# yzang2019/tendermint-fork

Hardware: AMD Instinct MI355X
Metric: ed25519 verifies/sec at 1/8 MI355X (higher is better)
Workload: dtype u32 (GF(2^255-19) radix 2^25.5 limbs, int64 accumulate); 1 GPU; C2: raw batch of 1048576 ed25519 signatures per GPU; signatures_per_gpu=1048576, key_cache=False, parallelism=shard-per-gpu x1

## Files before the change

### include/tmed25519.h

```cpp
#ifndef TMED25519_H
#define TMED25519_H

#include <stddef.h>
#include <stdint.h>

#ifdef __cplusplus
extern "C" {
#endif

#define TMED_OK 0
#define TMED_EINVAL (-1)
#define TMED_ENODEV (-2)
#define TMED_EHIP (-3)
#define TMED_ENOMEM (-4)
#define TMED_ENOKEYSET (-5)
#define TMED_EINTERNAL (-6)

typedef struct tmed_ctx tmed_ctx;

int tmed_device_count(void);

int tmed_init(int device, tmed_ctx **out);
void tmed_destroy(tmed_ctx *ctx);
const char *tmed_strerror(int code);
// ... 35 lines not shown
                                    const uint8_t *d_msgs, const uint32_t *d_msg_off, size_t n, uint8_t *d_out_valid,
                                    void *stream);


int tmed_verify_batch_zip215(tmed_ctx *ctx, const uint8_t *pubkeys, const uint8_t *sigs, const uint32_t *sig_lens,
                             const uint8_t *msgs, const uint32_t *msg_off, size_t n, uint8_t *out_valid);
int tmed_verify_batch_zip215_device(tmed_ctx *ctx, const uint8_t *d_pubkeys, const uint8_t *d_sigs,
                                    const uint8_t *d_msgs, const uint32_t *d_msg_off, size_t n, uint8_t *d_out_valid,
                                    void *stream);
int tmed_zip215_set_seed(const uint8_t *seed32);
int tmed_zip215_stats(uint32_t out[4]);


typedef struct {
  const char *chain_id;
  uint32_t chain_id_len;
  int64_t height;
  int32_t round;
  const uint8_t *block_hash;
  uint32_t block_hash_len;
  uint32_t psh_total;
  const uint8_t *psh_hash;
  uint32_t psh_hash_len;
} tmed_vote_template;

int tmed_vote_sign_bytes(const tmed_vote_template *t, size_t n, const uint8_t *flags, const int64_t *ts_seconds,
                         const int32_t *ts_nanos, uint8_t *out, size_t out_cap, uint32_t *out_off, size_t *out_len);


int tmed_valu_peak(tmed_ctx *ctx, int kind, double *giga_ops_per_s);

void tmed_test_pool_jitter(int max_us);
void tmed_test_stream_delay(int us);

int tmed_debug_zero_bits(void *out, size_t cap, size_t *n);


typedef struct {
  const uint8_t *hash;
  uint32_t hash_len;
  uint32_t psh_total;
  const uint8_t *psh_hash;
  uint32_t psh_hash_len;
} tmed_block_id;

typedef struct {
  size_t n;
  const uint8_t *pubkeys;
  const int64_t *powers;
  const uint8_t *addresses;
  int64_t total_power;
  uint64_t keyset;
  const uint32_t *keyset_index;
  const uint8_t *set_hash;
} tmed_valset;

typedef struct {
  int64_t height;
  int32_t round;
  tmed_block_id block_id;
  size_t n_sigs;
  const uint8_t *flags;
  const uint8_t *addresses;
  const int64_t *ts_seconds;
  const int32_t *ts_nanos;
  const uint8_t *sigs;
// ... 223 lines not shown
```

### tendermint-fork_amd/csrc/kernels.h

```cpp
#pragma once
#include <hip/hip_runtime.h>
#include <stddef.h>
#include <stdint.h>

#include "ge25519.h"
#include "signbytes.h"

namespace tmed {

struct KernelTimer {
  static constexpr int kMax = 160;
  hipEvent_t ev[kMax];
  int kind[kMax];
  int n = 0;
  void mark(hipStream_t s, int k) {
    if (n < kMax) { kind[n] = k; (void)hipEventRecord(ev[n++], s); }
  }
};

constexpr uint32_t kThreadsPerBlock = 256;
constexpr uint32_t kSlabSlotBytes = 8 * 128;
inline uint32_t slab_tables(int main_waves) { return main_waves == 5 ? 1u : 2u; }

constexpr uint32_t kFinCap = 1u << 20;
constexpr int kFinInt4 = 8;
constexpr uint32_t kFinGroupMax = 16;
constexpr uint32_t kFinPreStride = kFinCap + 64;
constexpr size_t kFinBytes = (size_t)kFinCap * kFinInt4 * 16;
constexpr size_t kFinPreBytes = (size_t)kFinPreStride * 3 * 16;

struct BTabs {
  const int4 *b16;
  const int4 *comb16;
  const int4 *b26 = nullptr;
};
constexpr uint32_t kB26Entries = (1u << 25) + 1;
constexpr size_t kB26Bytes = 2 * (size_t)kB26Entries * 128;
hipError_t launch_build_b26(const int4 *comb16, int4 *tab, hipStream_t stream);
constexpr int kB24Windows = 11;
constexpr uint32_t kB24Entries = (1u << 23) + 1;
constexpr size_t kB24Bytes = (size_t)kB24Windows * kB24Entries * 128;
hipError_t launch_build_b24(const int4 *comb16, int4 *tab, hipStream_t stream);
constexpr uint32_t kB16Entries = 32769;
constexpr size_t kB16Bytes = (size_t)kB16Entries * 128;
hipError_t launch_build_b16(int4 *tab, hipStream_t stream);
constexpr size_t kBComb16Bytes = 16 * kB16Bytes;
void host_bcomb16_bases(int32_t out[16 * 40]);
hipError_t launch_build_bcomb16(const int32_t *d_bases, int4 *comb, hipStream_t stream);

hipError_t launch_verify(const uint8_t *pub, const uint8_t *sig, const uint8_t *msgs, const uint32_t *off,
                         uint32_t n, uint8_t *out, int4 *slab, uint32_t slab_stride, BTabs btab,
                         int4 *prep, int4 *fin, int4 *fin_pre, hipStream_t stream, uint32_t chunk = 0,
                         int main_waves = 6, bool msg_slots = false, KernelTimer *timer = nullptr,
                         bool zip215 = false);

// ... 17 lines not shown
constexpr uint32_t kKeyChunksMax = (1u << 24) >> kKeyChunkBits;

hipError_t launch_comb_bases(const uint8_t *pubs, uint32_t n, int negate, uint8_t *ok, int32_t *bases,
                             hipStream_t stream);
hipError_t launch_comb_fill(const int32_t *bases, uint32_t n, int4 *comb, hipStream_t stream);
#ifndef TMED_COMBA_BITS
#define TMED_COMBA_BITS 12
#endif
constexpr int kCombABits = TMED_COMBA_BITS;
constexpr int kCombAWindows = 253 / kCombABits;
constexpr int kCombATopField = 253 - kCombABits * (kCombAWindows - 1);
constexpr uint32_t kCombAEntries = (1u << (kCombABits - 1)) + 1;
constexpr uint32_t kCombATopMax = (1u << (kCombATopField - 1)) + 1;
constexpr uint32_t kCombATopGroups = (kCombATopMax + 127) / 128;
constexpr uint32_t kCombATopEntries = kCombATopGroups * 128 + 1;
static_assert(kCombABits >= 10 && kCombABits <= 12 && kCombATopField >= kCombABits, "comb radix");
constexpr size_t kCombARowsPerKey = (size_t)(kCombAWindows - 1) * kCombAEntries + kCombATopEntries;
constexpr size_t kCombABytesPerKey = kCombARowsPerKey * kCombEntryInt4 * 16;
constexpr size_t comba_row(int w, uint32_t j) { return (size_t)w * kCombAEntries + j; }
hipError_t launch_build_comba(const uint8_t *pubs, uint32_t n, int32_t *bases, int4 *comba, hipStream_t stream);
hipError_t launch_verify_keyset(const uint32_t *val_idx, uint32_t nkeys, const uint8_t *key_pub, const uint8_t *key_ok,
                                const int4 *const *acomb, const int4 *bcomb, const uint8_t *sig, const uint8_t *msgs,
                                const uint32_t *off, uint32_t n, uint8_t *out, int4 *prep, uint32_t stride,
                                int4 *fin, int4 *fin_pre, hipStream_t stream, bool msg_slots = false,
                                KernelTimer *timer = nullptr, uint32_t *perm = nullptr,
                                uint32_t *order_scratch = nullptr, const int4 *bcomb24 = nullptr,
                                const int4 *const *acomba = nullptr);
constexpr uint32_t kKeyOrderMaxKeys = 1u << 24;
uint32_t key_order_scratch_words(uint32_t n, uint32_t nkeys);
hipError_t launch_key_order(const uint32_t *val_idx, uint32_t n, uint32_t nkeys, uint32_t *scratch, uint32_t *perm,
                            uint32_t index_base, hipStream_t stream);

hipError_t launch_test_delay(hipStream_t stream, uint32_t us);
hipError_t launch_window_stats(const int4 *prep, uint32_t stride, uint32_t count, uint32_t *d_hist,
                               hipStream_t stream);

constexpr uint32_t kLatMax = 1u << 16;
struct VoteAsm;
hipError_t launch_verify_keyset_lat(const uint32_t *val_idx, uint32_t nkeys, const uint8_t *key_pub, const uint8_t *key_ok,
                                    const int4 *const *acomb, const int4 *bcomb, const uint8_t *sig, const uint8_t *msgs,
                                    const uint32_t *off, uint32_t n, uint8_t *out, int4 *fin, int4 *dec,
                                    hipStream_t stream, bool msg_slots = false, const VoteAsm *va = nullptr);

constexpr uint32_t kGLatMax = 1u << 16;
constexpr size_t kGLatHandBytes = (size_t)kGLatMax * (6 * 2 + 7) * 16;
struct VoteAsm {
  const uint8_t *tmpl;
  const uint32_t *tmpl_idx;
  const uint8_t *flags;
  const int64_t *ts_sec;
  const int32_t *ts_nanos;
};

hipError_t launch_verify_glat(const uint8_t *pub, const uint8_t *sig, const uint8_t *msgs, const uint32_t *off,
                              uint32_t n, uint8_t *out, const int4 *comb16, int4 *hand, hipStream_t stream,
                              bool msg_slots = false, KernelTimer *timer = nullptr, const VoteAsm *va = nullptr);

hipError_t launch_assemble_votes(const uint8_t *tmpl, const uint32_t *tmpl_idx, const uint8_t *flags,
                                 const int64_t *ts_sec, const int32_t *ts_nanos, uint32_t n, uint8_t *out,
                                 uint32_t *out_len, hipStream_t stream);

}
```

### tendermint-fork_amd/csrc/kernels.hip

```cpp
#include "kernels.h"
#include "verify_core.h"
#include "verify_hs.h"
#include "kernel_util.h"
#include "rows.h"
#include "votes_dev.h"

namespace tmed {

__device__ int4 kIdentityRow[8] = {{1, 0, 0, 0}, {0, 0, 0, 0}, {1, 0, 0, 0}, {0, 0, 0, 0},
                                          {1, 0, 0, 0}, {0, 0, 0, 0}, {0, 0, 0, 0}, {0, 0, 0, 0}};

__device__ __forceinline__ void slab_st(int4 *p, int4 v) { *p = v; }
__device__ __forceinline__ int4 slab_ld(const int4 *p) { return *p; }

struct SlabTab {
  int4 *base;
  uint32_t slot;

  __device__ __forceinline__ const int4 *row(int j) const {
    return j == 0 ? kIdentityRow : base + ((size_t)slot * 8 + (j - 1)) * 8;
  }

  __device__ __forceinline__ void store(int j, const ge_cached &c) const {
    if (j == 0) return;
    int4 *r = base + ((size_t)slot * 8 + (j - 1)) * 8;
    const fe *fs[4] = {&c.YpX, &c.YmX, &c.Z, &c.T2d};
#pragma unroll
    for (int f = 0; f < 4; f++) {
      uint32_t w[8];
      fe_pack256(w, *fs[f]);
      slab_st(r + 2 * f, make_int4((int)w[0], (int)w[1], (int)w[2], (int)w[3]));
      slab_st(r + 2 * f + 1, make_int4((int)w[4], (int)w[5], (int)w[6], (int)w[7]));
    }
  }
  int4 pv[8];
  __device__ __forceinline__ void prefetch(int j, bool swap = false) {
    const int4 *r = row(j);
    const int sx = swap ? 2 : 0;
#pragma unroll
    for (int q = 0; q < 8; q++) pv[q] = slab_ld(r + (q < 4 ? (q ^ sx) : q));
  }
  __device__ __forceinline__ void take(ge_cached &c) const {
    fe *fs[4] = {&c.YpX, &c.YmX, &c.Z, &c.T2d};
#pragma unroll
    for (int f = 0; f < 4; f++) {
      const uint32_t w[8] = {(uint32_t)pv[2 * f].x, (uint32_t)pv[2 * f].y, (uint32_t)pv[2 * f].z,
                             (uint32_t)pv[2 * f].w, (uint32_t)pv[2 * f + 1].x, (uint32_t)pv[2 * f + 1].y,
                             (uint32_t)pv[2 * f + 1].z, (uint32_t)pv[2 * f + 1].w};
      fe_unpack256(*fs[f], w);
    }
  }
};

typedef __attribute__((address_space(1))) void global_void;
typedef __attribute__((address_space(3))) void lds_void;

template <int BITS>
struct BPf {
  static constexpr int kBits = BITS;
  const int4 *tab;
  int4 *buf;
  uint32_t lane;
  __device__ __forceinline__ void prefetch(int j) const {
    __builtin_amdgcn_s_waitcnt(0xc07f);
#pragma unroll
    for (int q = 0; q < 8; q++)
      __builtin_amdgcn_global_load_lds((global_void *)(tab + (size_t)j * 8 + q), (lds_void *)(buf + q * 64), 16, 0, 0);
  }
  __device__ __forceinline__ void take(ge_niels &e) const { niels_load(e, buf + lane, 64); }
};

constexpr uint32_t kHsBlock = kThreadsPerBlock;

constexpr int kPrepWaves = 3;
__global__ __launch_bounds__(kHsBlock, kPrepWaves) void verify_prep_kernel(
    const uint8_t *__restrict__ pub, const uint8_t *__restrict__ sig, MsgSrc ms, uint32_t base, uint32_t count,
    int4 *__restrict__ prep, uint32_t stride, uint32_t *__restrict__ place) {
  const uint32_t slot = blockIdx.x * blockDim.x + threadIdx.x;
  if (place && slot == 0) place[0] = place[1] = 0;
  if (slot >= count) return;
  const uint32_t i = base + slot;
  uint32_t pw[8];
  bool sok;
  {
    uint32_t sw[16], k[8], h[16];
// ... 163 lines not shown
    const int4 v = active ? prep2[(size_t)q * stride + slot] : make_int4(0, 0, 0, 0);
    w[4 * q] = v.x; w[4 * q + 1] = v.y; w[4 * q + 2] = v.z; w[4 * q + 3] = v.w;
  }
  uint32_t er[8];
#pragma unroll
  for (int j = 0; j < 8; j++) er[j] = (uint32_t)w[13 + j];
  if (BB == 16) {
    uint32_t e[8];
#pragma unroll
    for (int j = 0; j < 8; j++) e[j] = er[j];
    sc_recode_b<16>(er, e);
  }
  fe Rx, Ry;
#pragma unroll
  for (int j = 0; j < 10; j++) { Rx.v[j] = w[21 + j]; Ry.v[j] = w[31 + j]; }
  ge_p3 A;
#pragma unroll
  for (int j = 0; j < 10; j++) { A.X.v[j] = w[44 + j]; A.Y.v[j] = w[54 + j]; }
  if (!active) { fe_1(A.Y); fe_1(Ry); }
  fe_1(A.Z);
  fe_mul(A.T, A.X, A.Y);
  const int flags = w[41];
  int W = active ? (flags >> 8) : 29;
#pragma unroll
  for (int o = 32; o > 0; o >>= 1) {
    const int x = __shfl_xor(W, o);
    W = x > W ? x : W;
  }
  W = __builtin_amdgcn_readfirstlane(W);
  if (W < 29) W = 29;
  if (W > 64) W = 64;
  const uint32_t lane = threadIdx.x & 63u, wv = threadIdx.x >> 6;
  const HsDigitsDev ds{prep2, stride, slot, active};
  SlabTab ta{slab, slot};
  SlabTab tr{slab + (size_t)stride * 64, slot};
  const size_t hi = BB == 26 ? (size_t)kB26Entries * kCombEntryInt4 : (size_t)8 * kB16Entries * kCombEntryInt4;
  BPf<BB> bl{btab, sbl[wv], lane};
  BPf<BB> bh{btab + hi, sbh[wv], lane};
  const bool id = verify_main_hs(ds, (flags & 2) != 0, er, W, A, Rx, Ry, ta, tr, bl, bh, zip215 != 0);
  if (active) out[base + (uint32_t)w[42]] = ((flags & 1) && id) ? 1 : 0;
}

__global__ __launch_bounds__(kThreadsPerBlock) void window_stats_kernel(const int4 *__restrict__ prep2, uint32_t stride,
                                                                       uint32_t count, uint32_t *__restrict__ lane_hist,
                                                                       uint32_t *__restrict__ wave_hist) {
  __shared__ uint32_t lh[65], wh[65];
  for (uint32_t b = threadIdx.x; b < 65; b += blockDim.x) lh[b] = wh[b] = 0;
  __syncthreads();
  const uint32_t slot = blockIdx.x * blockDim.x + threadIdx.x;
  const bool active = slot < count;
  int W = active ? (prep2[(size_t)10 * stride + slot].y >> 8) : 0;
  if (W < 0 || W > 64) W = 64;
  if (active) atomicAdd(&lh[W], 1u);
  int m = W;
#pragma unroll
  for (int o = 32; o > 0; o >>= 1) {
    const int x = __shfl_xor(m, o);
    m = x > m ? x : m;
  }
  if ((threadIdx.x & 63u) == 0 && slot < count) atomicAdd(&wh[m], 1u);
  __syncthreads();
  for (uint32_t b = threadIdx.x; b < 65; b += blockDim.x) {
    if (lh[b]) atomicAdd(&lane_hist[b], lh[b]);
    if (wh[b]) atomicAdd(&wave_hist[b], wh[b]);
  }
}

__global__ __launch_bounds__(64) void test_delay_kernel(uint32_t iters) {
  for (uint32_t i = 0; i < iters; i++) __builtin_amdgcn_s_sleep(127);
}

hipError_t launch_test_delay(hipStream_t stream, uint32_t us) {
  if (us == 0) return hipSuccess;
  hipLaunchKernelGGL(test_delay_kernel, dim3(1), dim3(64), 0, stream, (us < 100000u ? us : 100000u) / 3u + 1u);
  return hipGetLastError();
}

hipError_t launch_window_stats(const int4 *prep, uint32_t stride, uint32_t count, uint32_t *d_hist,
                               hipStream_t stream) {
  if (count == 0) return hipSuccess;
  hipError_t e = hipMemsetAsync(d_hist, 0, 2 * 65 * sizeof(uint32_t), stream);
  if (e != hipSuccess) return e;
  hipLaunchKernelGGL(window_stats_kernel, dim3((count + kThreadsPerBlock - 1) / kThreadsPerBlock),
                     dim3(kThreadsPerBlock), 0, stream, prep + (size_t)kPrepInt4 * stride, stride, count, d_hist,
                     d_hist + 65);
  return hipGetLastError();
}

struct FinDev {
  const int4 *fin;
  int4 *pre;
  const uint8_t *sig;
  uint8_t *out;
  uint32_t fin_base, lane, L, m;
  const uint32_t *perm;
  __device__ __forceinline__ int count() const { return lane < m ? (int)((m - lane + L - 1) / L) : 0; }
  __device__ __forceinline__ uint32_t slot(int j) const { return lane + (uint32_t)j * L; }
  __device__ __forceinline__ void load_z(int j, fe &z) const {
// ... 697 lines not shown
```

### tendermint-fork_amd/csrc/tmed_capi.hip

```cpp
#include <hip/hip_runtime.h>
#include <stdlib.h>
#include <string.h>

#include <algorithm>
#include <map>
#include <mutex>
#include <new>
#include <string>

#include "../../include/tmed25519.h"
#include "kernels.h"

#include "ctx.h"
#include "median_host.h"

using namespace tmed;

extern "C" {

int tmed_device_count(void) {
  int n = 0;
  if (hipGetDeviceCount(&n) != hipSuccess) return 0;
  return n;
}
// ... 88 lines not shown

int tmed_init(int device, tmed_ctx **out) {
  if (!out) return TMED_EINVAL;
  *out = nullptr;
  int ndev = tmed_device_count();
  if (device < 0 || device >= ndev) return TMED_ENODEV;
  hipDeviceProp_t prop;
  if (hipGetDeviceProperties(&prop, device) != hipSuccess) return TMED_EHIP;
  if (strncmp(prop.gcnArchName, "gfx950", 6) != 0) return TMED_ENODEV;
  if (hipSetDevice(device) != hipSuccess) return TMED_EHIP;
  tmed_ctx *c = new tmed_ctx();
  c->device = device;
  hipError_t e = hipStreamCreateWithFlags(&c->stream, hipStreamNonBlocking);
  if (e == hipSuccess) e = hipStreamCreateWithFlags(&c->copy_stream, hipStreamNonBlocking);
  if (e == hipSuccess) e = hipEventCreate(&c->ev0);
  if (e == hipSuccess) e = hipEventCreate(&c->ev1);
  if (e == hipSuccess) e = hipEventCreateWithFlags(&c->scratch_ev, hipEventDisableTiming);
  auto round_up = [](uint32_t v) {
    if (v < kThreadsPerBlock) v = kThreadsPerBlock;
    if (v > (1u << 24)) v = 1u << 24;
    return (v + kThreadsPerBlock - 1) / kThreadsPerBlock * kThreadsPerBlock;
  };
  c->slab_slots = 4096 * kThreadsPerBlock;
  c->chunk = c->slab_slots;
  if (const char *v = getenv("TMED_SLAB_SLOTS")) c->slab_slots = round_up((uint32_t)strtoul(v, nullptr, 10));
  c->chunk = c->slab_slots;
  if (const char *v = getenv("TMED_CHUNK")) c->chunk = std::min(c->slab_slots, round_up((uint32_t)strtoul(v, nullptr, 10)));
  if (const char *v = getenv("TMED_MAIN_WAVES")) c->main_waves = atoi(v) == 5 ? 5 : 6;
  if (const char *v = getenv("TMED_LAT_MAX")) c->lat_max = (uint32_t)strtoul(v, nullptr, 10);
  if (c->lat_max > kLatMax) c->lat_max = kLatMax;
  if (const char *v = getenv("TMED_GLAT_MAX")) c->glat_max = (uint32_t)strtoul(v, nullptr, 10);
  if (c->glat_max > kGLatMax) c->glat_max = kGLatMax;
  if (e == hipSuccess)
    e = hipMalloc((void **)&c->d_slab, (size_t)c->slab_slots * kSlabSlotBytes * slab_tables(c->main_waves));
  if (e == hipSuccess) e = hipMalloc((void **)&c->d_prep, (size_t)c->slab_slots * kPrepSlotBytes + kPrepTailBytes);
  if (e == hipSuccess) e = hipMalloc((void **)&c->d_fin, kFinBytes);
  if (e == hipSuccess) e = hipMalloc((void **)&c->d_fin_pre, kFinPreBytes);
  if (e == hipSuccess) e = hipMalloc((void **)&c->d_glat, kGLatHandBytes);
  uint8_t *d_bpub = nullptr, *d_bok = nullptr;
  const uint8_t benc[32] = {0x58, 0x66, 0x66, 0x66, 0x66, 0x66, 0x66, 0x66, 0x66, 0x66, 0x66,
                            0x66, 0x66, 0x66, 0x66, 0x66, 0x66, 0x66, 0x66, 0x66, 0x66, 0x66,
                            0x66, 0x66, 0x66, 0x66, 0x66, 0x66, 0x66, 0x66, 0x66, 0x66};
  if (e == hipSuccess) e = hipMalloc((void **)&c->d_b16, kB16Bytes);
  if (e == hipSuccess) e = launch_build_b16(c->d_b16, c->stream);
  if (e == hipSuccess) e = hipMalloc((void **)&c->d_bcomb16, kBComb16Bytes);
  {
    static int32_t bases[16 * 40];
    static std::once_flag bases_once;
    std::call_once(bases_once, [] { host_bcomb16_bases(bases); });
    int32_t *d_bases = nullptr;
    if (e == hipSuccess) e = hipMalloc((void **)&d_bases, sizeof(bases));
    if (e == hipSuccess) e = hipMemcpy(d_bases, bases, sizeof(bases), hipMemcpyHostToDevice);
    if (e == hipSuccess) e = launch_build_bcomb16(d_bases, c->d_bcomb16, c->stream);
    if (e == hipSuccess) e = hipStreamSynchronize(c->stream);
    if (d_bases) (void)hipFree(d_bases);
  }
  if (e == hipSuccess && !env_off("TMED_B26")) c->d_b26 = bshare_acquire(0, device, c->d_bcomb16, c->stream);
  c->b24_on = !env_off("TMED_B24");
  c->acomb_on = !env_off("TMED_KS_ACOMB");
  if (const char *v = getenv("TMED_TEST_FAIL_KS_ALLOC")) c->test_fail_ks_alloc = atoi(v);
  c->kc_on = !env_off("TMED_KEYCACHE");
  if (const char *v = getenv("TMED_KEYCACHE_GB")) c->kc_budget = (size_t)strtoull(v, nullptr, 10) << 30;
  if (e == hipSuccess) e = hipMalloc((void **)&c->d_bcomb, kCombBytesPerKey);
  if (e == hipSuccess) e = hipMalloc((void **)&d_bpub, 32);
  if (e == hipSuccess) e = hipMalloc((void **)&d_bok, 1);
  if (e == hipSuccess) e = hipMemcpy(d_bpub, benc, 32, hipMemcpyHostToDevice);
  int rc = map_err(e);
// ... 197 lines not shown
  } else if (radix_bits == kCombABits) {
    if (k->comba.empty() || key >= k->comba_n || window >= (uint32_t)kCombAWindows) return TMED_EINVAL;
    if (j >= (window + 1 == (uint32_t)kCombAWindows ? kCombATopEntries : kCombAEntries)) return TMED_EINVAL;
    src = k->comba_row_of(key, comba_row((int)window, j));
  } else {
    return TMED_EINVAL;
  }
  int4 row[kCombEntryInt4];
  if (hipStreamSynchronize(c->stream) != hipSuccess || hipDeviceSynchronize() != hipSuccess) return TMED_EHIP;
  if (hipMemcpy(row, src, sizeof(row), hipMemcpyDeviceToHost) != hipSuccess) return TMED_EHIP;
  const int32_t *w = reinterpret_cast<const int32_t *>(row);
  for (int i = 0; i < 30; i++) out[i] = w[i];
  return TMED_OK;
}

int tmed_window_stats(tmed_ctx *c, uint32_t lane_hist[65], uint32_t wave_hist[65]) {
  if (!c || !lane_hist || !wave_hist) return TMED_EINVAL;
  std::lock_guard<std::mutex> lk(c->mu);
  for (int w = 0; w < 65; w++) lane_hist[w] = wave_hist[w] = 0;
  if (c->last_hs_count == 0) return TMED_OK;
  (void)hipSetDevice(c->device);
  uint32_t *d = nullptr;
  hipError_t e = hipMalloc((void **)&d, 2 * 65 * sizeof(uint32_t));
  if (e == hipSuccess) e = scratch_acquire(c, c->stream);
  if (e == hipSuccess) e = launch_window_stats(c->d_prep, c->slab_slots, c->last_hs_count, d, c->stream);
  if (e == hipSuccess) e = scratch_release(c, c->stream);
  uint32_t h[130];
  if (e == hipSuccess) e = hipMemcpyAsync(h, d, sizeof h, hipMemcpyDeviceToHost, c->stream);
  if (e == hipSuccess) e = hipStreamSynchronize(c->stream);
  if (d) (void)hipFree(d);
  if (e != hipSuccess) return map_err(e);
  for (int w = 0; w < 65; w++) { lane_hist[w] = h[w]; wave_hist[w] = h[65 + w]; }
  return TMED_OK;
}

int tmed_sign_batch_device(tmed_ctx *c, const uint8_t *d_seeds, const uint8_t *d_msgs, const uint32_t *d_off,
                           size_t n, uint8_t *d_sig_out, uint8_t *d_pub_out, void *stream) {
  if (!c) return TMED_EINVAL;
  if (n == 0) return TMED_OK;
  if (!d_seeds || !d_msgs || !d_off || !d_sig_out || !d_pub_out || n > 0xffffffffu) return TMED_EINVAL;
  hipStream_t s = stream ? (hipStream_t)stream : c->stream;
  hipSetDevice(c->device);
  return map_err(launch_sign(d_seeds, d_msgs, d_off, (uint32_t)n, d_sig_out, d_pub_out, c->d_bcomb, s));
}

static int check_offsets(const uint32_t *off, size_t n) {
  for (size_t i = 0; i < n; i++)
    if (off[i + 1] < off[i]) return TMED_EINVAL;
  return TMED_OK;
}

int tmed_verify_batch(tmed_ctx *c, const uint8_t *pub, const uint8_t *sig, const uint32_t *sig_lens,
                      const uint8_t *msgs, const uint32_t *off, size_t n, uint8_t *out) {
  if (!c || !out) return TMED_EINVAL;
  if (n == 0) return TMED_OK;
  if (!pub || !sig || !off || n > 0xffffffffu) return TMED_EINVAL;
  if (check_offsets(off, n) != TMED_OK) return TMED_EINVAL;
  const size_t mbytes = off[n];
  if (mbytes && !msgs) return TMED_EINVAL;
  std::lock_guard<std::mutex> lk(c->mu);
  hipSetDevice(c->device);
  hipError_t e = hipSuccess;
  const size_t moff_bytes = (n + 1) * 4;
  for (auto &pr : {std::make_pair(&c->d_a, n * 32), std::make_pair(&c->d_b, n * 64),
                   std::make_pair(&c->d_msg, mbytes + 16), std::make_pair(&c->d_off, moff_bytes),
                   std::make_pair(&c->d_out, n)})
// ... 71 lines not shown
```

### tendermint-fork_amd/csrc/verify_core.h

```cpp
#pragma once
#include "ge25519.h"
#include "sc25519.h"
#include "sha512.h"

namespace tmed {

TMED_HD void sc_recode256(uint32_t r[8], const uint32_t k[8]) {
  uint64_t c = 0;
#pragma unroll
  for (int i = 0; i < 8; i++) {
    const uint64_t t = (uint64_t)k[i] + 0x80808080u + c;
    r[i] = (uint32_t)t;
    c = t >> 32;
  }
}

TMED_HD void niels_apply_sign(ge_niels &e, bool neg) {
  fe t;
  fe_copy(t, e.YpX);
  fe_select(e.YpX, e.YpX, e.YmX, neg);
  fe_select(e.YmX, e.YmX, t, neg);
  fe_neg(t, e.XY2d);
  fe_select(e.XY2d, e.XY2d, t, neg);
}
// ... 13 lines not shown
  for (int j = 2; j <= 8; j++) {
    ge_add_cached(t, cur, c1, false);
    ge_p1p1_to_p3(cur, t);
    ge_p3_to_cached(c, cur);
    tab.store(j, c);
  }
}

template <class T>
TMED_HD void build_table_affine(T &tab, const ge_p3 &P) {
  ge_cached c;
  ge_cached_0(c);
  tab.store(0, c);
  fe d2;
  fe_const_d2(d2);
  ge_niels n;
  fe_add(n.YpX, P.Y, P.X);
  fe_sub(n.YmX, P.Y, P.X);
  fe_mul(n.XY2d, P.T, d2);
  fe_copy(c.YpX, n.YpX);
  fe_copy(c.YmX, n.YmX);
  fe_1(c.Z);
  fe_copy(c.T2d, n.XY2d);
  tab.store(1, c);
  ge_p3 cur = P;
  ge_p1p1 t;
#pragma unroll 1
  for (int j = 2; j <= 8; j++) {
    ge_madd_niels(t, cur, n, false);
    ge_p1p1_to_p3(cur, t);
    ge_p3_to_cached(c, cur);
    tab.store(j, c);
  }
}

template <int BBITS>
TMED_HD void sc_recode_b(uint32_t r[8], const uint32_t s[8]) {
  uint64_t c = 0;
#pragma unroll
  for (int i = 0; i < 8; i++) {
    const uint64_t t = (uint64_t)s[i] + (BBITS == 8 ? 0x80808080u : 0x80008000u) + c;
    r[i] = (uint32_t)t;
    c = t >> 32;
  }
}

template <int BBITS, class T, class BT>
TMED_HD void double_scalarmult(ge_p2 &out, const uint32_t k[8], const uint32_t s[8], T &tab, BT &btab) {
  constexpr int kBias = 1 << (BBITS - 1);
  constexpr uint32_t kMask = (1u << BBITS) - 1u;
  uint32_t kr[8], sr[8];
  sc_recode16(kr, k);
  sc_recode_b<BBITS>(sr, s);
  ge_p2 q;
  ge_p2_0(q);
  ge_p1p1 t;
  ge_p3 r;
  ge_cached ca;
  ge_niels nb;
  {
    const int da0 = (int)(kr[7] >> 28) - 8;
    tab.prefetch(da0 < 0 ? -da0 : da0);
    const int db0 = (int)(sr[7] >> (32 - BBITS)) - kBias;
    btab.prefetch(db0 < 0 ? -db0 : db0);
  }
#pragma unroll 1
// ... 440 lines not shown
```

### tendermint-fork_amd/csrc/verify_hs.h

```cpp
#pragma once
#include <math.h>

#include "verify_core.h"

namespace tmed {

TMED_HD void sc_const_8L(uint32_t n[8]) {
  const uint32_t c[8] = {0xe7ae9f68u, 0xc09318d2u, 0x17bce6b2u, 0xa6f7cef5u, 0u, 0u, 0u, 0x80000000u};
#pragma unroll
  for (int i = 0; i < 8; i++) n[i] = c[i];
}

TMED_HD int bitlen_words(const uint32_t *x, int n) {
  int b = 0;
#pragma unroll
  for (int i = 0; i < n; i++)
    if (x[i]) b = 32 * i + 32 - __builtin_clz(x[i]);
  return b;
}

TMED_HD double words_to_double(const uint32_t *x, int n) {
  double r = 0.0;
#pragma unroll
  for (int i = n - 1; i >= 0; i--) r = r * 4294967296.0 + (double)x[i];
// ... 338 lines not shown
      ge_p2_dbl(t, q);
      ge_p1p1_to_p3(r, t);
      ta.take(ca);
      tr.prefetch(dd < 0 ? -dd : dd, dd < 0);
      ge_add_cached_pre(t, r, ca, dc < 0);
      ge_p1p1_to_p3(r, t);
      tr.take(ca);
      ge_add_cached_pre(t, r, ca, dd < 0);
    }
    if (b26) {
      if (n == 0 || n == 13 || n == 26) hs_b26_add(t, r, n / 13 * 2, d26l, d26h, bl, bh);
    } else if ((n & 3) == 0 && n <= 28) {
      const int dl = (int)(el[3] >> 16) - 32768, dh = (int)(eh[3] >> 16) - 32768;
      words4_shl16(el);
      words4_shl16(eh);
      ge_p1p1_to_p3(r, t);
      bl.take(nb);
      const int nl = (int)(el[3] >> 16) - 32768;
      bl.prefetch(nl < 0 ? -nl : nl);
      niels_apply_sign(nb, dl < 0);
      ge_madd_niels(t, r, nb, false);
      ge_p1p1_to_p3(r, t);
      bh.take(nb);
      const int nh = (int)(eh[3] >> 16) - 32768;
      bh.prefetch(nh < 0 ? -nh : nh);
      niels_apply_sign(nb, dh < 0);
      ge_madd_niels(t, r, nb, false);
    }
    ge_p1p1_to_p2(q, t);
  }
  out = q;
}

TMED_HD bool p2_is_identity(const ge_p2 &q) { return fe_iszero(q.X) && fe_equal(q.Y, q.Z) && !fe_iszero(q.Z); }

TMED_HD void p2_mul8(ge_p2 &q) {
  ge_p1p1 t;
#pragma unroll 1
  for (int i = 0; i < 3; i++) {
    ge_p2_dbl(t, q);
    ge_p1p1_to_p2(q, t);
  }
}

template <class DS, class TA, class TR, class BL, class BH>
TMED_HD bool verify_main_hs(const DS &ds, bool dneg, const uint32_t er[8], int W, const ge_p3 &A, const fe &Rx,
                            const fe &Ry, TA &ta, TR &tr, BL &bl, BH &bh, bool cofactor8 = false) {
  ge_p3 P;
  fe_neg(P.X, A.X);
  fe_copy(P.Y, A.Y);
  fe_1(P.Z);
  fe_neg(P.T, A.T);
  build_table_affine(ta, P);
  if (dneg) fe_copy(P.X, Rx); else fe_neg(P.X, Rx);
  fe_copy(P.Y, Ry);
  fe_mul(P.T, P.X, P.Y);
  build_table_affine(tr, P);
  ge_p2 q;
  hs_straus(q, ds, er, W, ta, tr, bl, bh);
  if (cofactor8) p2_mul8(q);
  return p2_is_identity(q);
}

}
```

### tendermint-fork_amd/tmed/_native.py

```python
from __future__ import annotations

import ctypes
import os

PKG_ROOT = os.path.dirname(os.path.dirname(os.path.abspath(__file__)))
LIB_PATH = os.environ.get("TMED_LIB") or os.path.join(PKG_ROOT, "lib", "libtmed25519_hip.so")

TMED_OK = 0
TMED_EINVAL = -1
TMED_ENODEV = -2
TMED_EHIP = -3
TMED_ENOMEM = -4
TMED_ENOKEYSET = -5
TMED_EINTERNAL = -6

_lib = None


class TmedError(RuntimeError):
    def __init__(self, code: int, what: str = ""):
        self.code = code
        msg = lib().tmed_strerror(code).decode() if _lib is not None else str(code)
        super().__init__("%s: %s (code %d)" % (what or "tmed", msg, code))

# ... 50 lines not shown
    l.tmed_set_kernel_timing.restype = I
    l.tmed_set_kernel_timing.argtypes = [P, I]
    l.tmed_kernel_times.restype = I
    l.tmed_kernel_times.argtypes = [P, ctypes.POINTER(ctypes.c_float), ctypes.POINTER(ctypes.c_int)]
    l.tmed_last_kernel_ms.restype = ctypes.c_float
    l.tmed_last_kernel_ms.argtypes = [P]
    l.tmed_window_stats.restype = I
    l.tmed_window_stats.argtypes = [P, P, P]
    l.tmed_b_window_bits.restype = I
    l.tmed_b_window_bits.argtypes = [P]
    l.tmed_keyset_b_window_bits.restype = I
    l.tmed_keyset_b_window_bits.argtypes = [P]
    l.tmed_keyset_a_window_bits.restype = I
    l.tmed_keyset_a_window_bits.argtypes = [P, ctypes.c_uint64]
    l.tmed_keyset_comb_entry.restype = I
    l.tmed_keyset_comb_entry.argtypes = [P, ctypes.c_uint64, ctypes.c_uint32, ctypes.c_int, ctypes.c_uint32,
                                         ctypes.c_uint32, P]
    l.tmed_host_alloc.restype = I
    l.tmed_host_alloc.argtypes = [SZ, ctypes.POINTER(ctypes.c_void_p)]
    l.tmed_host_free.restype = I
    l.tmed_host_free.argtypes = [P]
    l.tmed_host_register.restype = I
    l.tmed_host_register.argtypes = [P, SZ]
    l.tmed_host_unregister.restype = I
    l.tmed_host_unregister.argtypes = [P]
    l.tmed_verify_batch_zip215.argtypes = [P, P, P, P, P, P, SZ, P]
    l.tmed_verify_batch_zip215_device.argtypes = [P, P, P, P, P, SZ, P, P]
    l.tmed_zip215_set_seed.argtypes = [P]
    l.tmed_zip215_stats.argtypes = [P]
    l.tmed_test_pool_jitter.restype = None
    l.tmed_test_pool_jitter.argtypes = [I]
    l.tmed_test_stream_delay.restype = None
    l.tmed_test_stream_delay.argtypes = [I]
    l.tmed_debug_zero_bits.restype = I
    l.tmed_debug_zero_bits.argtypes = [P, SZ, ctypes.POINTER(SZ)]
    _lib = l
    return l


EXPORTED_SYMBOLS = [
    "tmed_device_count", "tmed_init", "tmed_destroy", "tmed_strerror",
    "tmed_verify_batch", "tmed_verify_batch_device",
    "tmed_sign_batch", "tmed_sign_batch_device", "tmed_last_kernel_ms",
    "tmed_vote_sign_bytes", "tmed_valu_peak", "tmed_verify_commits", "tmed_verify_commits_with",
    "tmed_test_pool_jitter", "tmed_test_stream_delay", "tmed_debug_zero_bits",
    "tmed_keyset_load", "tmed_keyset_free", "tmed_keyset_extend", "tmed_verify_batch_keyset",
    "tmed_keycache_config", "tmed_keycache_stats", "tmed_keycache_flush", "tmed_keycache_warm", "tmed_keycache_wait", "tmed_verify_batch_keyset_device",
    "tmed_set_kernel_timing", "tmed_kernel_times", "tmed_blocksync_verify", "tmed_blocksync_submit", "tmed_blocksync_wait",
    "tmed_merkle_roots", "tmed_valset_hashes", "tmed_header_hashes", "tmed_partset_roots",
    "tmed_commit_hashes", "tmed_txs_hashes",
    "tmed_merkle_proofs", "tmed_partset_proofs", "tmed_txs_proofs", "tmed_merkle_proofs_verify",
    "tmed_light_verify", "tmed_light_verify_with",
    "tmed_median_times", "tmed_median_times_host",
    "tmed_verify_commits_multi", "tmed_blocksync_verify_multi", "tmed_window_stats", "tmed_b_window_bits", "tmed_keyset_b_window_bits", "tmed_keyset_a_window_bits", "tmed_keyset_comb_entry", "tmed_seam_phase_us",
    "tmed_verify_batch_zip215", "tmed_verify_batch_zip215_device", "tmed_zip215_set_seed", "tmed_zip215_stats",
    "tmed_host_alloc", "tmed_host_free", "tmed_host_register", "tmed_host_unregister",
]
```

Measured before the change: 107.5 million verifies/s.

## Replace separate A/R Straus tables with a joint radix-4 combination table

Swaps the two independent per-signature precomputed tables for A and R in the half-size Straus verify for a single joint table of 12 cached rows holding i*P + j*Q for small digits. Each 4-bit window digit is split into a high and a low radix-4 part, so every pair of doublings is followed by one joint add instead of separate additions from two tables. This is meant to cut point additions in the main loop and shrink slab memory from two 8-row tables to one 12-row table, at the cost of a more involved table build and an extra add for the top digit. A test entry point that exports the joint rows is also added.

```diff
diff --git a/include/tmed25519.h b/include/tmed25519.h
--- a/include/tmed25519.h
+++ b/include/tmed25519.h
@@ -91,6 +91,9 @@
 
 void tmed_test_pool_jitter(int max_us);
 void tmed_test_stream_delay(int us);
+
+int tmed_test_joint_rows(tmed_ctx *ctx, const uint8_t *a, const uint8_t *r, const uint8_t *dneg, size_t n,
+                         uint8_t *rows);
 
 int tmed_debug_zero_bits(void *out, size_t cap, size_t *n);
 
diff --git a/tendermint-fork_amd/csrc/kernels.h b/tendermint-fork_amd/csrc/kernels.h
--- a/tendermint-fork_amd/csrc/kernels.h
+++ b/tendermint-fork_amd/csrc/kernels.h
@@ -20,7 +20,8 @@
 
 constexpr uint32_t kThreadsPerBlock = 256;
 constexpr uint32_t kSlabSlotBytes = 8 * 128;
-inline uint32_t slab_tables(int main_waves) { return main_waves == 5 ? 1u : 2u; }
+constexpr uint32_t kSlabJointSlotBytes = 12 * 128;
+inline size_t slab_bytes(uint32_t slots) { return (size_t)slots * kSlabJointSlotBytes; }
 
 constexpr uint32_t kFinCap = 1u << 20;
 constexpr int kFinInt4 = 8;
@@ -104,6 +105,8 @@
                             uint32_t index_base, hipStream_t stream);
 
 hipError_t launch_test_delay(hipStream_t stream, uint32_t us);
+hipError_t launch_test_joint_rows(const uint8_t *a, const uint8_t *r, const uint8_t *dneg, uint32_t n, int4 *rows,
+                                  hipStream_t stream);
 hipError_t launch_window_stats(const int4 *prep, uint32_t stride, uint32_t count, uint32_t *d_hist,
                                hipStream_t stream);
 
diff --git a/tendermint-fork_amd/csrc/kernels.hip b/tendermint-fork_amd/csrc/kernels.hip
--- a/tendermint-fork_amd/csrc/kernels.hip
+++ b/tendermint-fork_amd/csrc/kernels.hip
@@ -13,17 +13,18 @@
 __device__ __forceinline__ void slab_st(int4 *p, int4 v) { *p = v; }
 __device__ __forceinline__ int4 slab_ld(const int4 *p) { return *p; }
 
-struct SlabTab {
+template <int ROWS>
+struct SlabTabN {
   int4 *base;
   uint32_t slot;
 
   __device__ __forceinline__ const int4 *row(int j) const {
-    return j == 0 ? kIdentityRow : base + ((size_t)slot * 8 + (j - 1)) * 8;
+    return j == 0 ? kIdentityRow : base + ((size_t)slot * ROWS + (j - 1)) * 8;
   }
 
   __device__ __forceinline__ void store(int j, const ge_cached &c) const {
     if (j == 0) return;
-    int4 *r = base + ((size_t)slot * 8 + (j - 1)) * 8;
+    int4 *r = base + ((size_t)slot * ROWS + (j - 1)) * 8;
     const fe *fs[4] = {&c.YpX, &c.YmX, &c.Z, &c.T2d};
 #pragma unroll
     for (int f = 0; f < 4; f++) {
@@ -51,6 +52,9 @@
     }
   }
 };
+using SlabTab = SlabTabN<8>;
+using SlabTabJ = SlabTabN<kJointRows>;
+static_assert(kSlabSlotBytes == 8 * 128 && kSlabJointSlotBytes == kJointRows * 128, "slab rows are 128 B");
 
 typedef __attribute__((address_space(1))) void global_void;
 typedef __attribute__((address_space(3))) void lds_void;
@@ -280,12 +284,11 @@
   if (W > 64) W = 64;
   const uint32_t lane = threadIdx.x & 63u, wv = threadIdx.x >> 6;
   const HsDigitsDev ds{prep2, stride, slot, active};
-  SlabTab ta{slab, slot};
-  SlabTab tr{slab + (size_t)stride * 64, slot};
+  SlabTabJ tj{slab, slot};
   const size_t hi = BB == 26 ? (size_t)kB26Entries * kCombEntryInt4 : (size_t)8 * kB16Entries * kCombEntryInt4;
   BPf<BB> bl{btab, sbl[wv], lane};
   BPf<BB> bh{btab + hi, sbh[wv], lane};
-  const bool id = verify_main_hs(ds, (flags & 2) != 0, er, W, A, Rx, Ry, ta, tr, bl, bh, zip215 != 0);
+  const bool id = verify_main_hsj(ds, (flags & 2) != 0, er, W, A, Rx, Ry, tj, bl, bh, zip215 != 0);
   if (active) out[base + (uint32_t)w[42]] = ((flags & 1) && id) ? 1 : 0;
 }
 
@@ -312,6 +315,31 @@
     if (lh[b]) atomicAdd(&lane_hist[b], lh[b]);
     if (wh[b]) atomicAdd(&wave_hist[b], wh[b]);
   }
+}
+
+__global__ __launch_bounds__(kHsBlock) void test_joint_rows_kernel(const uint8_t *__restrict__ a,
+                                                                   const uint8_t *__restrict__ r,
+                                                                   const uint8_t *__restrict__ dneg, uint32_t n,
+                                                                   int4 *__restrict__ rows) {
+  const uint32_t i = blockIdx.x * blockDim.x + threadIdx.x;
+  if (i >= n) return;
+  uint32_t aw[8], rw[8];
+  load_row_words(aw, a + 32 * (size_t)i, 2);
+  load_row_words(rw, r + 32 * (size_t)i, 2);
+  ge_p3 A, R, P, Q;
+  ge_frombytes_go(A, aw);
+  ge_frombytes_go(R, rw);
+  hs_points(P, Q, dneg[i] != 0, A, R.X, R.Y);
+  SlabTabJ tj{rows, i};
+  build_table_joint(tj, P, Q);
+}
+
+hipError_t launch_test_joint_rows(const uint8_t *a, const uint8_t *r, const uint8_t *dneg, uint32_t n, int4 *rows,
+                                  hipStream_t stream) {
+  if (n == 0) return hipSuccess;
+  hipLaunchKernelGGL(test_joint_rows_kernel, dim3((n + kHsBlock - 1) / kHsBlock), dim3(kHsBlock), 0, stream, a, r,
+                     dneg, n, rows);
+  return hipGetLastError();
 }
 
 __global__ __launch_bounds__(64) void test_delay_kernel(uint32_t iters) {
diff --git a/tendermint-fork_amd/csrc/tmed_capi.hip b/tendermint-fork_amd/csrc/tmed_capi.hip
--- a/tendermint-fork_amd/csrc/tmed_capi.hip
+++ b/tendermint-fork_amd/csrc/tmed_capi.hip
@@ -144,7 +144,7 @@
   if (const char *v = getenv("TMED_GLAT_MAX")) c->glat_max = (uint32_t)strtoul(v, nullptr, 10);
   if (c->glat_max > kGLatMax) c->glat_max = kGLatMax;
   if (e == hipSuccess)
-    e = hipMalloc((void **)&c->d_slab, (size_t)c->slab_slots * kSlabSlotBytes * slab_tables(c->main_waves));
+    e = hipMalloc((void **)&c->d_slab, slab_bytes(c->slab_slots));
   if (e == hipSuccess) e = hipMalloc((void **)&c->d_prep, (size_t)c->slab_slots * kPrepSlotBytes + kPrepTailBytes);
   if (e == hipSuccess) e = hipMalloc((void **)&c->d_fin, kFinBytes);
   if (e == hipSuccess) e = hipMalloc((void **)&c->d_fin_pre, kFinPreBytes);
@@ -408,6 +408,28 @@
   if (e != hipSuccess) return map_err(e);
   for (int w = 0; w < 65; w++) { lane_hist[w] = h[w]; wave_hist[w] = h[65 + w]; }
   return TMED_OK;
+}
+
+int tmed_test_joint_rows(tmed_ctx *c, const uint8_t *a, const uint8_t *r, const uint8_t *dneg, size_t n,
+                         uint8_t *rows) {
+  if (!c || !a || !r || !dneg || !rows || n == 0 || n > 65536) return TMED_EINVAL;
+  std::lock_guard<std::mutex> lk(c->mu);
+  (void)hipSetDevice(c->device);
+  uint8_t *d_in = nullptr;
+  int4 *d_rows = nullptr;
+  const size_t row_bytes = n * kSlabJointSlotBytes;
+  hipError_t e = hipMalloc((void **)&d_in, 65 * n);
+  if (e == hipSuccess) e = hipMalloc((void **)&d_rows, row_bytes);
+  if (e == hipSuccess) e = hipMemcpyAsync(d_in, a, 32 * n, hipMemcpyHostToDevice, c->stream);
+  if (e == hipSuccess) e = hipMemcpyAsync(d_in + 32 * n, r, 32 * n, hipMemcpyHostToDevice, c->stream);
+  if (e == hipSuccess) e = hipMemcpyAsync(d_in + 64 * n, dneg, n, hipMemcpyHostToDevice, c->stream);
+  if (e == hipSuccess) e = launch_test_joint_rows(d_in, d_in + 32 * n, d_in + 64 * n, (uint32_t)n, d_rows, c->stream);
+  if (e == hipSuccess) e = hipMemcpyAsync(rows, d_rows, row_bytes, hipMemcpyDeviceToHost, c->stream);
+  const hipError_t es = hipStreamSynchronize(c->stream);
+  if (e == hipSuccess) e = es;
+  if (d_in) (void)hipFree(d_in);
+  if (d_rows) (void)hipFree(d_rows);
+  return e == hipSuccess ? TMED_OK : map_err(e);
 }
 
 int tmed_sign_batch_device(tmed_ctx *c, const uint8_t *d_seeds, const uint8_t *d_msgs, const uint32_t *d_off,
diff --git a/tendermint-fork_amd/csrc/verify_core.h b/tendermint-fork_amd/csrc/verify_core.h
--- a/tendermint-fork_amd/csrc/verify_core.h
+++ b/tendermint-fork_amd/csrc/verify_core.h
@@ -69,6 +69,120 @@
     ge_p3_to_cached(c, cur);
     tab.store(j, c);
   }
+}
+
+constexpr int kJointRows = 12;
+TMED_HD int joint_index(int i, int j) { return 5 * i + j; }
+
+TMED_HD void ge_affine_dbl(ge_p1p1 &r, const fe &s, const fe &d) {
+  fe S, D, M, four;
+  fe_sq_x2(S, s, D, d);
+  fe_mul(M, s, d);
+  fe_0(four);
+  four.v[0] = 4;
+  fe_sub(r.X, S, D);
+  fe_add(r.Y, S, D);
+  fe_add(r.Z, M, M);
+  fe_sub(r.T, four, r.Z);
+}
+
+template <bool FLIP>
+TMED_HD void ge_madd_niels_pm(ge_p1p1 &s, ge_p1p1 &m, const fe &t, const fe &t2, const fe &pT, const fe *pZ,
+                              const ge_niels &q) {
+  fe a, b, ap, bp, c, d;
+  fe_mul_x2(a, t, q.YpX, bp, t2, q.YpX);
+  fe_mul_x2(ap, t, q.YmX, b, t2, q.YmX);
+  fe_mul(c, q.XY2d, pT);
+  if (pZ) {
+    fe_add(d, *pZ, *pZ);
+  } else {
+    fe_0(d);
+    d.v[0] = 2;
+  }
+  fe_sub(s.X, a, b);
+  fe_add(s.Y, a, b);
+  fe_add(s.Z, d, c);
+  fe_sub(s.T, d, c);
+  if (FLIP) fe_sub(m.X, bp, ap); else fe_sub(m.X, ap, bp);
+  fe_add(m.Y, ap, bp);
+  fe_sub(m.Z, d, c);
+  fe_add(m.T, d, c);
+}
+template <bool FLIP>
+TMED_HD void ge_madd_niels_pm(ge_p1p1 &s, ge_p1p1 &m, const ge_p3 &p, const ge_niels &q) {
+  fe t, t2;
+  fe_add(t, p.Y, p.X);
+  fe_sub(t2, p.Y, p.X);
+  ge_madd_niels_pm<FLIP>(s, m, t, t2, p.T, &p.Z, q);
+}
+
+template <class T>
+TMED_HD void joint_store(T &tab, int row, ge_p3 &p, const ge_p1p1 &t) {
+  ge_cached c;
+  ge_p1p1_to_p3(p, t);
+  ge_p3_to_cached(c, p);
+  tab.store(row, c);
+}
+
+template <class T>
+TMED_HD void build_table_joint(T &tab, const ge_p3 &P, const ge_p3 &Q) {
+  ge_cached c;
+  ge_p1p1 s, m;
+  ge_p3 u;
+  ge_p2 v;
+  ge_niels n;
+  ge_cached_0(c);
+  tab.store(0, c);
+  {
+    fe d2, t, t2;
+    fe_const_d2(d2);
+    fe_add(t, P.Y, P.X);
+    fe_sub(t2, P.Y, P.X);
+    fe_add(n.YpX, Q.Y, Q.X);
+    fe_sub(n.YmX, Q.Y, Q.X);
+    fe_mul_x2(c.T2d, P.T, d2, n.XY2d, Q.T, d2);
+    fe_1(c.Z);
+    fe_copy(c.YpX, t);
+    fe_copy(c.YmX, t2);
+    tab.store(joint_index(1, 0), c);
+    fe_copy(c.YpX, n.YpX);
+    fe_copy(c.YmX, n.YmX);
+    fe_copy(c.T2d, n.XY2d);
+    tab.store(joint_index(0, 1), c);
+    ge_madd_niels_pm<false>(s, m, t, t2, P.T, nullptr, n);
+  }
+  joint_store(tab, joint_index(1, 1), u, s);
+  ge_p3_to_p2(v, u);
+  ge_p2_dbl(s, v);
+  joint_store(tab, joint_index(2, 2), u, s);
+  joint_store(tab, joint_index(1, -1), u, m);
+  ge_p3_to_p2(v, u);
+  ge_p2_dbl(s, v);
+  tab.prefetch(joint_index(0, 1), false);
+  joint_store(tab, joint_index(2, -2), u, s);
+  tab.take(c);
+  tab.prefetch(joint_index(1, 0), false);
+  ge_affine_dbl(s, c.YpX, c.YmX);
+  joint_store(tab, joint_index(0, 2), u, s);
+  tab.take(c);
+  fe_copy(n.YpX, c.YpX);
+  fe_copy(n.YmX, c.YmX);
+  fe_copy(n.XY2d, c.T2d);
+  ge_madd_niels_pm<true>(s, m, u, n);
+  joint_store(tab, joint_index(1, 2), u, s);
+  tab.prefetch(joint_index(1, 0), false);
+  joint_store(tab, joint_index(1, -2), u, m);
+  tab.take(c);
+  tab.prefetch(joint_index(0, 1), false);
+  ge_affine_dbl(s, c.YpX, c.YmX);
+  joint_store(tab, joint_index(2, 0), u, s);
+  tab.take(c);
+  fe_copy(n.YpX, c.YpX);
+  fe_copy(n.YmX, c.YmX);
+  fe_copy(n.XY2d, c.T2d);
+  ge_madd_niels_pm<false>(s, m, u, n);
+  joint_store(tab, joint_index(2, 1), u, s);
+  joint_store(tab, joint_index(2, -1), u, m);
 }
 
 template <int BBITS>
diff --git a/tendermint-fork_amd/csrc/verify_hs.h b/tendermint-fork_amd/csrc/verify_hs.h
--- a/tendermint-fork_amd/csrc/verify_hs.h
+++ b/tendermint-fork_amd/csrc/verify_hs.h
@@ -394,6 +394,109 @@
   out = q;
 }
 
+TMED_HD void hs_split4(int D, int &h, int &l) {
+  l = ((D + 2) & 3) - 2;
+  h = (D - l) >> 2;
+}
+
+template <class DS, class TJ, class BL, class BH>
+TMED_HD void hs_straus_joint(ge_p2 &out, const DS &ds, const uint32_t er[8], int W, TJ &tj, BL &bl, BH &bh) {
+  constexpr bool b26 = BL::kBits == 26;
+  static_assert(BL::kBits == 16 || BL::kBits == 26, "B windows of radix 2^16 or 2^26");
+  uint32_t el[4] = {er[0], er[1], er[2], er[3]}, eh[4] = {er[4], er[5], er[6], er[7]};
+  int d26l[5] = {0, 0, 0, 0, 0}, d26h[5] = {0, 0, 0, 0, 0};
+  if (b26) {
+    hs_b26_digits(d26l, d26h, er);
+    bl.prefetch(d26l[4] < 0 ? -d26l[4] : d26l[4]);
+    bh.prefetch(d26h[4] < 0 ? -d26h[4] : d26h[4]);
+  } else {
+    const int dl = (int)(el[3] >> 16) - 32768, dh = (int)(eh[3] >> 16) - 32768;
+    bl.prefetch(dl < 0 ? -dl : dl);
+    bh.prefetch(dh < 0 ? -dh : dh);
+  }
+  ge_p2 q;
+  ge_p1p1 t;
+  ge_p3 r;
+  ge_cached ca;
+  ge_niels nb;
+  uint32_t cw = ds.cword((W - 1) >> 3), dw = ds.dword((W - 1) >> 3), cwn = cw, dwn = dw;
+  int ih = 0, il;
+  {
+    const int dc = hs_top_digit(cw, W < 64 ? ((W & 7) ? cw : ds.cword(W >> 3)) : 0u, W);
+    const int dd = hs_top_digit(dw, W < 64 ? ((W & 7) ? dw : ds.dword(W >> 3)) : 0u, W);
+    int hc, lc, hd, ld;
+    hs_split4(dc, hc, lc);
+    hs_split4(dd, hd, ld);
+    const int c1 = hc < 2 ? hc : 2, d1 = hd < 2 ? hd : 2;
+    tj.prefetch(joint_index(c1, d1), false);
+    tj.take(ca);
+    tj.prefetch(joint_index(hc - c1, hd - d1), false);
+    ge_cached_to_p3(r, ca);
+    tj.take(ca);
+    il = joint_index(lc, ld);
+    tj.prefetch(il < 0 ? -il : il, il < 0);
+    ge_add_cached_pre(t, r, ca, false);
+    ge_p1p1_to_p2(q, t);
+  }
+#pragma unroll 1
+  for (int n = W - 1; n >= 0; n--) {
+    if (n > 0 && ((n - 1) & 7) == 7) {
+      cwn = ds.cword((n - 1) >> 3);
+      dwn = ds.dword((n - 1) >> 3);
+    }
+    if (n != W - 1) {
+      ge_p2_dbl(t, q);
+      ge_p1p1_to_p2(q, t);
+      ge_p2_dbl(t, q);
+      ge_p1p1_to_p3(r, t);
+      tj.take(ca);
+      tj.prefetch(il < 0 ? -il : il, il < 0);
+      ge_add_cached_pre(t, r, ca, ih < 0);
+      if (b26 && (n == 6 || n == 19)) hs_b26_add(t, r, n == 19 ? 3 : 1, d26l, d26h, bl, bh);
+      ge_p1p1_to_p2(q, t);
+    }
+    ge_p2_dbl(t, q);
+    ge_p1p1_to_p2(q, t);
+    ge_p2_dbl(t, q);
+    ge_p1p1_to_p3(r, t);
+    tj.take(ca);
+    const bool lneg = il < 0;
+    if (n > 0) {
+      cw = cwn;
+      dw = dwn;
+      const int sh = 4 * ((n - 1) & 7);
+      int hc, lc, hd, ld;
+      hs_split4((int)((cw >> sh) & 15u) - 8, hc, lc);
+      hs_split4((int)((dw >> sh) & 15u) - 8, hd, ld);
+      ih = joint_index(hc, hd);
+      il = joint_index(lc, ld);
+      tj.prefetch(ih < 0 ? -ih : ih, ih < 0);
+    }
+    ge_add_cached_pre(t, r, ca, lneg);
+    if (b26) {
+      if (n == 0 || n == 13 || n == 26) hs_b26_add(t, r, n / 13 * 2, d26l, d26h, bl, bh);
+    } else if ((n & 3) == 0 && n <= 28) {
+      const int dl = (int)(el[3] >> 16) - 32768, dh = (int)(eh[3] >> 16) - 32768;
+      words4_shl16(el);
+      words4_shl16(eh);
+      ge_p1p1_to_p3(r, t);
+      bl.take(nb);
+      const int nl = (int)(el[3] >> 16) - 32768;
+      bl.prefetch(nl < 0 ? -nl : nl);
+      niels_apply_sign(nb, dl < 0);
+      ge_madd_niels(t, r, nb, false);
+      ge_p1p1_to_p3(r, t);
+      bh.take(nb);
+      const int nh = (int)(eh[3] >> 16) - 32768;
+      bh.prefetch(nh < 0 ? -nh : nh);
+      niels_apply_sign(nb, dh < 0);
+      ge_madd_niels(t, r, nb, false);
+    }
+    ge_p1p1_to_p2(q, t);
+  }
+  out = q;
+}
+
 TMED_HD bool p2_is_identity(const ge_p2 &q) { return fe_iszero(q.X) && fe_equal(q.Y, q.Z) && !fe_iszero(q.Z); }
 
 TMED_HD void p2_mul8(ge_p2 &q) {
@@ -405,23 +508,46 @@
   }
 }
 
-template <class DS, class TA, class TR, class BL, class BH>
-TMED_HD bool verify_main_hs(const DS &ds, bool dneg, const uint32_t er[8], int W, const ge_p3 &A, const fe &Rx,
-                            const fe &Ry, TA &ta, TR &tr, BL &bl, BH &bh, bool cofactor8 = false) {
-  ge_p3 P;
+TMED_HD void hs_points(ge_p3 &P, ge_p3 &Q, bool dneg, const ge_p3 &A, const fe &Rx, const fe &Ry) {
   fe_neg(P.X, A.X);
   fe_copy(P.Y, A.Y);
   fe_1(P.Z);
   fe_neg(P.T, A.T);
-  build_table_affine(ta, P);
-  if (dneg) fe_copy(P.X, Rx); else fe_neg(P.X, Rx);
-  fe_copy(P.Y, Ry);
-  fe_mul(P.T, P.X, P.Y);
-  build_table_affine(tr, P);
+  if (dneg) fe_copy(Q.X, Rx); else fe_neg(Q.X, Rx);
+  fe_copy(Q.Y, Ry);
+  fe_1(Q.Z);
+  fe_mul(Q.T, Q.X, Q.Y);
+}
+
+template <class DS, class TJ, class BL, class BH>
+TMED_HD bool verify_main_hsj(const DS &ds, bool dneg, const uint32_t er[8], int W, const ge_p3 &A, const fe &Rx,
+                             const fe &Ry, TJ &tj, BL &bl, BH &bh, bool cofactor8 = false) {
+  ge_p3 P, Q;
+  hs_points(P, Q, dneg, A, Rx, Ry);
+  build_table_joint(tj, P, Q);
   ge_p2 q;
-  hs_straus(q, ds, er, W, ta, tr, bl, bh);
+  hs_straus_joint(q, ds, er, W, tj, bl, bh);
   if (cofactor8) p2_mul8(q);
   return p2_is_identity(q);
 }
 
-}
+template <class TA, class TR>
+struct HsJointPair {
+  TA &ta;
+  TR &tr;
+  bool hi = false;
+  TMED_HDM void store(int j, const ge_cached &c) { if (j <= 8) ta.store(j, c); else tr.store(j - 8, c); }
+  TMED_HDM void prefetch(int j, bool swap = false) {
+    hi = j > 8;
+    if (hi) tr.prefetch(j - 8, swap); else ta.prefetch(j, swap);
+  }
+  TMED_HDM void take(ge_cached &c) const { if (hi) tr.take(c); else ta.take(c); }
+};
+template <class DS, class TA, class TR, class BL, class BH>
+TMED_HD bool verify_main_hs(const DS &ds, bool dneg, const uint32_t er[8], int W, const ge_p3 &A, const fe &Rx,
+                            const fe &Ry, TA &ta, TR &tr, BL &bl, BH &bh, bool cofactor8 = false) {
+  HsJointPair<TA, TR> tj{ta, tr};
+  return verify_main_hsj(ds, dneg, er, W, A, Rx, Ry, tj, bl, bh, cofactor8);
+}
+
+}
diff --git a/tendermint-fork_amd/tmed/_native.py b/tendermint-fork_amd/tmed/_native.py
--- a/tendermint-fork_amd/tmed/_native.py
+++ b/tendermint-fork_amd/tmed/_native.py
@@ -106,6 +106,8 @@
     l.tmed_test_pool_jitter.argtypes = [I]
     l.tmed_test_stream_delay.restype = None
     l.tmed_test_stream_delay.argtypes = [I]
+    l.tmed_test_joint_rows.restype = I
+    l.tmed_test_joint_rows.argtypes = [P, P, P, P, SZ, P]
     l.tmed_debug_zero_bits.restype = I
     l.tmed_debug_zero_bits.argtypes = [P, SZ, ctypes.POINTER(SZ)]
     _lib = l
@@ -117,7 +119,7 @@
     "tmed_verify_batch", "tmed_verify_batch_device",
     "tmed_sign_batch", "tmed_sign_batch_device", "tmed_last_kernel_ms",
     "tmed_vote_sign_bytes", "tmed_valu_peak", "tmed_verify_commits", "tmed_verify_commits_with",
-    "tmed_test_pool_jitter", "tmed_test_stream_delay", "tmed_debug_zero_bits",
+    "tmed_test_pool_jitter", "tmed_test_stream_delay", "tmed_test_joint_rows", "tmed_debug_zero_bits",
     "tmed_keyset_load", "tmed_keyset_free", "tmed_keyset_extend", "tmed_verify_batch_keyset",
     "tmed_keycache_config", "tmed_keycache_stats", "tmed_keycache_flush", "tmed_keycache_warm", "tmed_keycache_wait", "tmed_verify_batch_keyset_device",
     "tmed_set_kernel_timing", "tmed_kernel_times", "tmed_blocksync_verify", "tmed_blocksync_submit", "tmed_blocksync_wait",
```

After: 109.9 million verifies/s (median of 6 runs). 2.2% higher.
